# PRBonn/OverlapNet

Measured on NVIDIA H100. Metric: scan-pairs/sec (overlap+yaw) at 64x900, higher is better.
Workload: dtype f16

## Files before the change

overlapnet_b200/csrc/api.cu:

```cuda
#include "common.cuh"
#include <math.h>
#include <string.h>

using namespace ovn;

static const char* kLegNames[] = {"s_conv1", "s_conv2", "s_conv3", "s_conv3a", "s_conv4", "s_conv5",
                                  "s_conv6", "s_conv7", "s_conv8", "s_conv9", "s_conv10"};

static void set_spec(ConvSpec& L, const char* name, int kh, int kw, int sh, int sw, int cin, int cout, int relu,
                     int h_in, int w_in) {
  memset(&L, 0, sizeof(L));
  snprintf(L.name, sizeof(L.name), "%s", name);
  L.kh = kh; L.kw = kw; L.sh = sh; L.sw = sw; L.cin = cin; L.cout = cout; L.relu = relu;
  L.h_in = h_in; L.w_in = w_in;
  L.h_out = (h_in - kh) / sh + 1;
  L.w_out = (w_in - kw) / sw + 1;
}

static void slot_sizes(const ovn_handle* h, int slot, int64_t* n_kernel, int64_t* n_bias) {
  if (slot == kMaxLegLayers + 3) {
    *n_kernel = h->dense_in; *n_bias = 1;
    return;
  }
  const ConvSpec& L = slot < kMaxLegLayers ? h->leg[slot] : h->head[slot - kMaxLegLayers];
  *n_kernel = (int64_t)L.kh * L.kw * L.cin * L.cout;
  *n_bias = L.cout;
}

static __global__ void k_iota(int32_t* p, int n, int start) {
  const int i = blockIdx.x * blockDim.x + threadIdx.x;
  if (i < n) p[i] = start + i;
}

static __global__ void k_sanitize_idx(const int32_t* __restrict__ in, int32_t* __restrict__ out, int n, int64_t limit,
                                      int code, const int32_t* __restrict__ row_bad, int* __restrict__ err) {
  const int i = blockIdx.x * blockDim.x + threadIdx.x;
  if (i >= n) return;
  int64_t v = in[i];
  if (v < 0 || v >= limit) {
    atomicCAS(err, 0, code);
    v = v < 0 ? 0 : limit - 1;
  }
  if (row_bad && row_bad[v]) atomicCAS(err, 0, kErrNonFiniteOperand);
  out[i] = (int32_t)v;
}

struct PeerPtrs { int32_t* p[16]; };

static __global__ void k_peer_signal(PeerPtrs dst, int n, int value) {
  const int i = threadIdx.x;
  if (i >= n || dst.p[i] == nullptr) return;
  __threadfence_system();
  asm volatile("st.release.sys.global.s32 [%0], %1;" :: "l"(dst.p[i]), "r"(value) : "memory");
}

static __global__ void k_peer_wait(const int32_t* __restrict__ flags, int n, int skip, int value, int* __restrict__ err) {
  const int i = threadIdx.x;
  if (i >= n || i == skip) return;
  const long long t0 = clock64();
  for (;;) {
    int v;
    asm volatile("ld.acquire.sys.global.s32 %0, [%1];" : "=r"(v) : "l"(flags + i) : "memory");
    if (v >= value) break;
    if (clock64() - t0 > (1ll << 32)) { atomicCAS(err, 0, kErrPeerWait); break; }
    __nanosleep(32);
  }
}

namespace ovn {

int sanitize_indices(ovn_handle* h, const int32_t* d_in, int n, int64_t limit, int code, int32_t* d_out, cudaStream_t s,
                     const int32_t* row_bad) {
  if (n <= 0) return OVN_OK;
  k_sanitize_idx<<<(n + 255) / 256, 256, 0, s>>>(d_in, d_out, n, limit < 1 ? 1 : limit, code, row_bad, h->d_err);
  OVN_LAUNCH_CHECK(h);
  return OVN_OK;
}

int check_device_error(ovn_handle* h, cudaStream_t s) {
  if (!h->h_pinned || !h->d_err) return OVN_OK;
  int32_t* hp = &h->stage()->err;
  OVN_CUDA(h, cudaMemcpyAsync(hp, h->d_err, sizeof(int), cudaMemcpyDeviceToHost, s));
  OVN_CUDA(h, cudaStreamSynchronize(s));
  const int e = *hp;
  if (e == 0) return OVN_OK;
  OVN_CUDA(h, cudaMemsetAsync(h->d_err, 0, sizeof(int), s));
  const char* ring = nullptr;
  switch (e) {
    case kErrBadIndex: OVN_SET_ERR(h, OVN_ERR_INVALID_ARG, "a pair / candidate index is outside [0, bank_size)");
    case kErrRowNotPrepared:
      OVN_SET_ERR(h, OVN_ERR_INVALID_ARG, "resident bank: an indexed row was never passed to ovn_bank_prepare");
    case kErrNonFiniteOperand:
      OVN_SET_ERR(h, OVN_ERR_INVALID_ARG, "a feature volume value is not finite in the fp16 operands of the tensor-core "
                  "heads (NaN, inf, or |x - centre| > 65504); outputs of the call are poisoned (NaN / INT32_MIN)");
    case kErrPeerWait: OVN_SET_ERR(h, OVN_ERR_CUDA, "ovn_peer_wait timed out: a peer rank never signalled");
    case kErrInjectedFault: OVN_SET_ERR(h, OVN_ERR_CUDA, "tensor-core pipeline failed: k_conv2_wgmma: fault injected by "
                                        "OVN_DEBUG_FAULT (code %d); outputs of the call are poisoned (NaN / INT32_MIN)", e);
    case kErrDeltaLeftProducer: case kErrDeltaLeftConsumer: ring = "k_delta_conv1_wgmma: LEFT volume ring"; break;
    case kErrDeltaRightProducer: case kErrDeltaRightConsumer: ring = "k_delta_conv1_wgmma: RIGHT window ring"; break;
    case kErrDeltaW1Producer: case kErrDeltaW1Consumer: ring = "k_delta_conv1_wgmma: W1 ring"; break;
    case kErrConv2Producer: case kErrConv2Consumer: ring = "k_conv2_wgmma: o1 + W2 ring"; break;
    case kErrConv3X3Producer: case kErrConv3X3Consumer: ring = "k_conv3_wgmma: x3 ring"; break;
    case kErrConv3W3Producer: case kErrConv3W3Consumer: ring = "k_conv3_wgmma: W3 ring"; break;
    case kErrCorrRightProducer: case kErrCorrRightConsumer: ring = "k_corr_wgmma: RIGHT third ring"; break;
    case kErrCorrLeftProducer: case kErrCorrLeftConsumer: ring = "k_corr_wgmma: LEFT tile ring"; break;
  }
  if (!ring) OVN_SET_ERR(h, OVN_ERR_CUDA, "unknown device error code %d", e);
  OVN_SET_ERR(h, OVN_ERR_CUDA, "tensor-core pipeline failed: %s, %s wait timed out (code %d); outputs of the call are "
              "poisoned (NaN / INT32_MIN)", ring, e < 200 ? "producer" : "consumer", e);
}

}

extern "C" {

int ovn_abi_version(void) { return OVN_ABI_VERSION; }

const char* ovn_status_string(int status) {
  switch (status) {
    case OVN_OK: return "OVN_OK";
    case OVN_ERR_INVALID_ARG: return "OVN_ERR_INVALID_ARG";
    case OVN_ERR_BAD_CONFIG: return "OVN_ERR_BAD_CONFIG";
    case OVN_ERR_WEIGHTS: return "OVN_ERR_WEIGHTS";
    case OVN_ERR_CUDA: return "OVN_ERR_CUDA";
    case OVN_ERR_NO_DEVICE: return "OVN_ERR_NO_DEVICE";
    case OVN_ERR_CAPACITY: return "OVN_ERR_CAPACITY";
    default: return "OVN_ERR_UNKNOWN";
  }
}

void ovn_default_config(ovn_config* c) {
  if (!c) return;
  memset(c, 0, sizeof(*c));
  c->abi_version = OVN_ABI_VERSION;
  c->proj_H = 64; c->proj_W = 900;
  c->fov_up_deg = 3.0f; c->fov_down_deg = -25.0f;
  c->max_range = 50.0f;
  c->use_depth = 1; c->use_normals = 1;
  c->n_prob_channels = 0; c->use_intensity = 0;
  c->strides_layer1[0] = 2; c->strides_layer1[1] = 2;
  c->additional_unsymmetric_layer3a = 1;
  c->leg_output_width = 360;
  c->conv1size = 15;
  c->precision = OVN_PREC_F16_TC;
  c->max_batch_scans = 16;
  c->max_batch_pairs = 1101;
}

static thread_local std::string g_create_error;

const char* ovn_last_error(const ovn_handle* h) { return h ? h->last_error.c_str() : g_create_error.c_str(); }
int64_t ovn_launch_count(const ovn_handle* h) { return h ? h->launches : 0; }
int ovn_input_channels(const ovn_handle* h) { return h ? h->C : 0; }
int ovn_feature_width(const ovn_handle* h) { return h ? h->cfg.leg_output_width : 0; }
int ovn_feature_channels(const ovn_handle* h) { return h ? kFeatC : 0; }

#define CREATE_FAIL(code, ...)                              \
  do {                                                      \
    char _b[512];                                           \
    snprintf(_b, sizeof(_b), __VA_ARGS__);                  \
    g_create_error = _b;                                    \
    return (code);                                          \
  } while (0)

#define CREATE_CUDA(call)                                                              \
  do {                                                                                 \
    cudaError_t _e = (call);                                                           \
    if (_e != cudaSuccess) {                                                           \
      cudaGetLastError();                                                              \
      CREATE_FAIL(OVN_ERR_CUDA, "%s: %s", #call, cudaGetErrorString(_e));              \
    }                                                                                  \
  } while (0)

#define CREATE_ALLOC(buf, bytes)                                                       \
  do {                                                                                 \
    if ((buf).ensure(h.get(), (bytes)) != OVN_OK) CREATE_FAIL(OVN_ERR_CUDA, "ovn_create: %s", h->last_error.c_str()); \
  } while (0)

ovn_handle::~ovn_handle() {
  if (ev_bank) cudaEventDestroy(ev_bank);
  if (own_stream) cudaStreamDestroy(own_stream);
  for (auto& v : prof_ev) for (cudaEvent_t e : v) cudaEventDestroy(e);
}

int ovn_create(const ovn_config* cfg, ovn_handle** out) {
  if (!cfg || !out) CREATE_FAIL(OVN_ERR_INVALID_ARG, "ovn_create: NULL argument");
  *out = nullptr;
  if (cfg->abi_version != OVN_ABI_VERSION)
    CREATE_FAIL(OVN_ERR_INVALID_ARG, "ovn_create: abi_version %d != %d", cfg->abi_version, OVN_ABI_VERSION);
  int ndev = 0;
  if (cudaGetDeviceCount(&ndev) != cudaSuccess || ndev == 0) {
    cudaGetLastError();
    CREATE_FAIL(OVN_ERR_NO_DEVICE, "ovn_create: no CUDA device visible (this library has no CPU fallback)");
  }
  int dev = 0;
  CREATE_CUDA(cudaGetDevice(&dev));
  cudaDeviceProp prop;
  CREATE_CUDA(cudaGetDeviceProperties(&prop, dev));
  if (prop.major != 9 || prop.minor != 0)
    CREATE_FAIL(OVN_ERR_NO_DEVICE, "ovn_create: device %d is sm_%d%d; this build targets sm_90a only", dev,
                prop.major, prop.minor);
  std::unique_ptr<ovn_handle> h(new ovn_handle());
  h->cfg = *cfg;
  h->device = dev;
  h->sm_count = prop.multiProcessorCount;
  const ovn_config& c = h->cfg;
  if (c.proj_H <= 0 || c.proj_W <= 0 || c.max_batch_scans <= 0 || c.max_batch_pairs <= 0)
    CREATE_FAIL(OVN_ERR_BAD_CONFIG, "ovn_create: non-positive size in config");
  if (c.n_prob_channels != 0 && c.n_prob_channels != 3 && c.n_prob_channels != 20)
    CREATE_FAIL(OVN_ERR_BAD_CONFIG, "ovn_create: n_prob_channels must be 0, 3 or 20 (infer.py:68-73)");
  h->C = (c.use_depth ? 1 : 0) + (c.use_normals ? 3 : 0) + c.n_prob_channels + (c.use_intensity ? 1 : 0);
  if (h->C <= 0) CREATE_FAIL(OVN_ERR_BAD_CONFIG, "ovn_create: no input channel enabled");

  struct { int kh, kw, sh, sw, cout; bool opt; } T[] = {
      {5, 15, c.strides_layer1[0], c.strides_layer1[1], 16, false}, {3, 15, 2, 1, 32, false},
      {3, 15, 2, 1, 64, false},  {3, 12, 2, 1, 64, true},           {2, 9, 2, 1, 128, false},
      {1, 9, 1, 1, 128, false},  {1, 9, 1, 1, 128, false},          {1, 9, 1, 1, 128, false},
      {1, 7, 1, 1, 128, false},  {1, 5, 1, 1, 128, false},          {1, 3, 1, 1, 128, false}};
  int hh = c.proj_H, ww = c.proj_W, cc = h->C;
  h->n_leg = 0;
  h->net_ok = true;
  char nb[256];
  for (int i = 0; i < 11 && h->net_ok; ++i) {
    if (T[i].opt && !c.additional_unsymmetric_layer3a) continue;
    if (T[i].sh <= 0 || T[i].sw <= 0 || hh < T[i].kh || ww < T[i].kw) {
      snprintf(nb, sizeof(nb), "layer %s does not fit its input %dx%d", kLegNames[i], hh, ww);
      h->net_ok = false; h->net_error = nb;
      break;
    }
    set_spec(h->leg[h->n_leg], kLegNames[i], T[i].kh, T[i].kw, T[i].sh, T[i].sw, cc, T[i].cout, 1, hh, ww);
    hh = h->leg[h->n_leg].h_out; ww = h->leg[h->n_leg].w_out; cc = T[i].cout;
    h->n_leg++;
  }
  const int Wf = c.leg_output_width, s = c.conv1size;
  if (h->net_ok && (hh != 1 || ww != c.leg_output_width || cc != kFeatC)) {
    snprintf(nb, sizeof(nb), "leg output is %dx%dx%d, expected 1x%dx%d (network.yml:77)", hh, ww, cc,
             c.leg_output_width, kFeatC);
    h->net_ok = false; h->net_error = nb;
  }
  if (h->net_ok && (s <= 0 || Wf % s != 0 || Wf / s < 3)) {
    snprintf(nb, sizeof(nb), "conv1size %d must divide leg_output_width %d", s, Wf);
    h->net_ok = false; h->net_error = nb;
  }
  if (!h->net_ok) { h->n_leg = 0; *out = nullptr; }
  if (h->net_ok) {
    set_spec(h->head[0], "c_conv1", 1, s, 1, s, kFeatC, 64, 0, Wf, Wf);
    set_spec(h->head[1], "c_conv2", s, 1, s, 1, 64, 128, 1, h->head[0].h_out, h->head[0].w_out);
    set_spec(h->head[2], "c_conv3", 3, 3, 1, 1, 128, 256, 1, h->head[1].h_out, h->head[1].w_out);
    h->o1_h = h->head[0].h_out; h->o1_w = h->head[0].w_out;
    h->o2_h = h->head[1].h_out; h->o2_w = h->head[1].w_out;
    h->o3_h = h->head[2].h_out; h->o3_w = h->head[2].w_out;
    h->dense_in = h->o3_h * h->o3_w * h->head[2].cout;
    ParamLayout& P = h->params;
// ... 932 lines not shown
```

overlapnet_b200/csrc/common.cuh:

```cuda
#pragma once
#include <cuda_runtime.h>
#include <cuda_fp16.h>
#include <stddef.h>
#include <stdint.h>
#include <stdio.h>
#include <memory>
#include <string>
#include <vector>
#include <map>

#include "../../include/ovn_b200.h"

struct ovn_handle;

namespace ovn {

template <class T, bool Pinned = false>
class Buffer {
 public:
  Buffer() = default;
  Buffer(Buffer&& o) noexcept { swap(o); }
  Buffer& operator=(Buffer&& o) noexcept {
    Buffer old(std::move(o));
    swap(old);
// ... 60 lines not shown
  int64_t n_kernel[kMaxLegLayers + 4] = {};
  int64_t n_head = 0;
  int64_t n_total = 0;
};
inline int flat_slot(int i) { return i < 4 ? kMaxLegLayers + i : i - 4; }

enum GradCover { kNoGrads = 0, kHeadGrads, kNetGrads };

struct TrainState {
  Buffer<float> x4;
  Buffer<float> dx3;
  Buffer<float> corr;
  Buffer<float> overlap;
  Buffer<float> dz;
  Buffer<int32_t> yaw;
  Buffer<float> w3t;
  Buffer<float> part;
  Buffer<float> grad;
  Buffer<float> accum;
  Buffer<float> loss;
  Buffer<float> chunk_loss;
  PinnedBuffer<float> chunk_loss_host;
  GradCover grads = kNoGrads;
  Buffer<float> images;
  Buffer<float> acts;
  Buffer<float> dact[2];
  Buffer<float> dfv_part;
  Buffer<float> dcorr;
  Buffer<int32_t> pair_rows;
  Buffer<float> wt;
  int64_t net_fv_off = 0;
  int net_np = 0;
};
}

struct ovn_handle {
  ovn_config cfg;
  int device = 0;
  int sm_count = 0;
  std::string last_error;
  int64_t launches = 0;

  int C = 0;
  int n_leg = 0;
  ovn::ConvSpec leg[ovn::kMaxLegLayers];
  ovn::ConvSpec head[3];
  int o1_h = 0, o1_w = 0;
  int o2_h = 0, o2_w = 0;
  int o3_h = 0, o3_w = 0;
  int dense_in = 0;
  ovn::ParamLayout params;

  std::map<std::string, ovn::LayerWeights> host_w;
  bool weights_ready = false;
  bool net_ok = false;
  std::string net_error;

  ovn::Buffer<float> d_w[ovn::kMaxLegLayers + 4];
  ovn::Buffer<float> d_b[ovn::kMaxLegLayers + 4];

  ovn::Buffer<unsigned long long> d_keys;
  ovn::Buffer<unsigned long long> d_pair_keys;
  ovn::Buffer<uint8_t> d_pair_prune;
  ovn::Buffer<uint32_t> d_valid_words;
  ovn::Buffer<uint32_t> d_word_prefix;
  ovn::Buffer<uint32_t> d_scan_tmp;
  ovn::Buffer<float> d_act[2];
  ovn::Buffer<float> d_input;
  ovn::Buffer<float> d_o1;
  ovn::Buffer<float> d_o2;
  ovn::Buffer<float> d_G;
  ovn::Buffer<int32_t> d_cand_idx;
  ovn::Buffer<int32_t> d_idx_san;
  ovn::Buffer<int> d_err;
  cudaEvent_t ev_bank = nullptr;
  ovn::Buffer<float> d_query_fv;
  ovn::Buffer<float> d_query_overlap;
  ovn::Buffer<int32_t> d_query_yaw;
  ovn::Buffer<float> d_stage_points;
  ovn::Buffer<int64_t> d_stage_offsets;
  ovn::PinnedBuffer<uint8_t> h_pinned;
  cudaStream_t own_stream = nullptr;
  bool profiling = false;
  std::vector<cudaEvent_t> prof_ev[ovn::kProfKinds];
  std::unique_ptr<ovn::TcState, ovn::TcStateDelete> tc;
  std::unique_ptr<ovn::TrainState> train;
  int32_t train_precision = OVN_TRAIN_FP32;
  bool train_tc = false;
  bool dgrad_tc_smem = false;

  ~ovn_handle();
  ovn::StageHeader* stage() const { return reinterpret_cast<ovn::StageHeader*>(h_pinned.get()); }
  int32_t* stage_cand_idx() const { return reinterpret_cast<int32_t*>(h_pinned + sizeof(ovn::StageHeader)); }
  float* stage_overlap() const { return reinterpret_cast<float*>(stage_cand_idx() + cfg.max_batch_pairs); }
  int32_t* stage_yaw() const { return reinterpret_cast<int32_t*>(stage_overlap() + cfg.max_batch_pairs); }
};

#define OVN_SET_ERR(h, code, ...)                                 \
  do {                                                            \
    char _buf[512];                                               \
    snprintf(_buf, sizeof(_buf), __VA_ARGS__);                    \
    (h)->last_error = _buf;                                       \
    return (code);                                                \
  } while (0)

#define OVN_CUDA(h, call)                                                                   \
  do {                                                                                      \
    cudaError_t _e = (call);                                                                \
    if (_e != cudaSuccess) {                                                                \
      cudaGetLastError();                                                                   \
      OVN_SET_ERR(h, OVN_ERR_CUDA, "%s failed at %s:%d: %s", #call, __FILE__, __LINE__,     \
                  cudaGetErrorString(_e));                                                  \
    }                                                                                       \
  } while (0)

#define OVN_LAUNCH_CHECK(h)                                                                 \
  do {                                                                                      \
    (h)->launches++;                                                                        \
    cudaError_t _e = cudaGetLastError();                                                    \
    if (_e != cudaSuccess) {                                                                \
      OVN_SET_ERR(h, OVN_ERR_CUDA, "kernel launch failed at %s:%d: %s", __FILE__, __LINE__, \
                  cudaGetErrorString(_e));                                                  \
    }                                                                                       \
  } while (0)

namespace ovn {

template <class T, bool Pinned>
int Buffer<T, Pinned>::ensure(ovn_handle* h, size_t bytes, size_t reserve) {
  if (bytes <= cap_) return OVN_OK;
  *this = {};
  if (reserve < bytes) reserve = bytes;
  void* p = nullptr;
  if (Pinned) OVN_CUDA(h, cudaHostAlloc(&p, reserve, cudaHostAllocDefault));
  else OVN_CUDA(h, cudaMalloc(&p, reserve));
  p_ = static_cast<T*>(p);
  cap_ = reserve;
  return OVN_OK;
}

struct DeviceGuard {
  int prev = -1;
  bool switched = false;
  explicit DeviceGuard(const ovn_handle* h) {
    if (h && cudaGetDevice(&prev) == cudaSuccess && prev != h->device) switched = cudaSetDevice(h->device) == cudaSuccess;
  }
  ~DeviceGuard() { if (switched) cudaSetDevice(prev); }
};

enum DeviceError : int {
  kErrDeltaLeftProducer = 101, kErrDeltaLeftConsumer = 402,
  kErrDeltaRightProducer = 103, kErrDeltaRightConsumer = 404,
  kErrDeltaW1Producer = 102, kErrDeltaW1Consumer = 202,
  kErrConv2Producer = 111, kErrConv2Consumer = 211,
  kErrConv3X3Producer = 121, kErrConv3X3Consumer = 221,
  kErrConv3W3Producer = 122, kErrConv3W3Consumer = 222,
  kErrCorrRightProducer = 131, kErrCorrRightConsumer = 231,
  kErrCorrLeftProducer = 132, kErrCorrLeftConsumer = 232,
  kErrInjectedFault = 501,
  kErrBadIndex = 900,
  kErrRowNotPrepared = 901,
  kErrNonFiniteOperand = 910,
  kErrPeerWait = 950,
};

inline void prof_mark(ovn_handle* h, int kind, cudaStream_t s) {
  if (!h->profiling) return;
  cudaEvent_t e;
  if (cudaEventCreate(&e) != cudaSuccess) return;
  cudaEventRecord(e, s);
  h->prof_ev[kind].push_back(e);
}

template <class T>
int upload_vec(ovn_handle* h, Buffer<T>& dst, const std::vector<T>& v) {
  dst = {};
  const int rc = dst.ensure(h, v.size() * sizeof(T));
  if (rc != OVN_OK) return rc;
  OVN_CUDA(h, cudaMemcpy(dst, v.data(), v.size() * sizeof(T), cudaMemcpyHostToDevice));
  return OVN_OK;
}

int project_batch(ovn_handle* h, const float* d_points, const int64_t* d_offsets, int n_scans,
                  int64_t n_total, float max_range, float* d_range, float* d_vertex,
                  float* d_intensity, int32_t* d_idx, cudaStream_t s);
int normals_batch(ovn_handle* h, const float* d_range, const float* d_vertex, int n_scans,
                  float* d_normal, cudaStream_t s);
int semantic_batch(ovn_handle* h, const int32_t* d_idx, const float* d_probs,
                   const int64_t* d_offsets, int n_scans, int n_classes, float* d_out,
                   cudaStream_t s);
int preprocess_batch(ovn_handle* h, const float* d_points, const int64_t* d_offsets, int n_scans,
                     int64_t n_total, const float* d_probs, float* d_input, cudaStream_t s);
int gt_range_batch(ovn_handle* h, const float* d_points, const int64_t* d_offsets, int n_scans, int64_t n_total,
                   const double* d_pose_ref, const double* d_pose_cur_inv, float max_range, float* d_range,
                   cudaStream_t s);
int gt_overlap_count(ovn_handle* h, const float* d_ref, const float* d_cur, int n_scans, int32_t* d_counts, cudaStream_t s);
int gt_scan_radius(ovn_handle* h, const float* d_points, const int64_t* d_offsets, int n_scans, double* d_radius,
                   cudaStream_t s);
int gt_pairs_count(ovn_handle* h, const float* d_points, const int64_t* h_offsets, int n_ref, const double* d_pose_ref,
                   const double* d_radius, const float* d_cur_range, const double* d_pose_cur_inv, int n_cur,
                   float max_range, int tile_cur, int tile_ref, int32_t* d_counts, int64_t ld_counts,
                   int64_t* d_n_pruned, cudaStream_t s);
int pack_input(ovn_handle* h, const float* d_depth, const float* d_normal, const float* d_prob,
               const float* d_intensity, int n_scans, float* d_input, cudaStream_t s);

int leg_forward_fp32(ovn_handle* h, const float* d_input, int n, float* d_fv, cudaStream_t s);
int heads_forward_fp32(ovn_handle* h, const float* d_bank, const float* d_query,
                       const int32_t* d_left, const int32_t* d_right, int n, float* d_overlap,
                       int32_t* d_yaw, float* d_corr, cudaStream_t s);

constexpr int kMaxSumParts = 64;

struct GradChunks {
  int n = 1;
  int off[kMaxSumParts + 1] = {};
  float* grad = nullptr;
  int64_t stride = 0;
  float* loss = nullptr;
  __host__ __device__ int size(int c) const { return off[c + 1] - off[c]; }
};

int train_alloc(ovn_handle* h);
int head_gradients_fp32(ovn_handle* h, const float* d_bank, const int32_t* left, const int32_t* right, int np,
                        const float* d_gt_overlap, const int32_t* d_gt_orientation, float min_overlap,
                        const GradChunks& ch, cudaStream_t s);
int net_gradients_fp32(ovn_handle* h, const float* d_images, const int32_t* left, const int32_t* right, int np,
                       const float* d_gt_overlap, const int32_t* d_gt_orientation, float min_overlap,
                       float* d_fv_grad, const GradChunks& ch, cudaStream_t s);
int net_max_pairs(const ovn_handle* h);
int64_t train_workspace_bytes(const ovn_handle* h, bool whole_network, int np);
int copy_net_volumes_fp32(ovn_handle* h, float* d_out, cudaStream_t s);
int adagrad_sum_fp32(ovn_handle* h, bool whole_network, const float* d_parts, int n_parts, const float* h_weights,
                     float lr, cudaStream_t s);
int gather_images(ovn_handle* h, const float* d_images, int64_t n_images, const int32_t* d_rows,
                  const int32_t* d_shift, const float* d_rot, int n, float* d_out, cudaStream_t s);

int corr_forward_fp32(ovn_handle* h, const float* d_bank, const float* d_query, const int32_t* left,
                      const int32_t* right, int np, int32_t* d_yaw, float* d_corr, cudaStream_t s);

int leg_forward_tc(ovn_handle* h, const float* d_input, int n, float* d_fv, cudaStream_t s);
int heads_forward_tc(ovn_handle* h, const float* d_bank, const float* d_query,
                     const int32_t* d_left, const int32_t* d_right, int n, float* d_overlap,
                     int32_t* d_yaw, float* d_corr, cudaStream_t s);
int tc_pack_weights(ovn_handle* h);
int tc_bank_prepare(ovn_handle* h, const float* d_bank, int64_t capacity, int64_t first, int64_t count, cudaStream_t s);
int tc_bank_release(ovn_handle* h, const float* d_bank);
int tc_set_center(ovn_handle* h, const float* h_mu);
int tc_get_center(ovn_handle* h, float* h_mu, int32_t* is_set);
int tc_calibrate(ovn_handle* h, const float* d_volume, cudaStream_t s);
int tc_copy_heads_stage(ovn_handle* h, int stage, int64_t first, int64_t count, float* d_out, cudaStream_t s);
int64_t tc_heads_stage_pairs(const ovn_handle* h);
int sanitize_indices(ovn_handle* h, const int32_t* d_in, int n, int64_t limit, int code, int32_t* d_out, cudaStream_t s,
                     const int32_t* row_bad = nullptr);
int check_device_error(ovn_handle* h, cudaStream_t s);

}
```

overlapnet_b200/csrc/hopper.cuh:

```cuda
#pragma once
#include <cuda_runtime.h>
#include <stdint.h>

namespace hopper {

__device__ __forceinline__ uint32_t smem_u32(const void* p) { return (uint32_t)__cvta_generic_to_shared(p); }

__device__ __forceinline__ void mbar_init(uint64_t* bar, uint32_t count) {
  asm volatile("mbarrier.init.shared::cta.b64 [%0], %1;" :: "r"(smem_u32(bar)), "r"(count) : "memory");
}
__device__ __forceinline__ void mbar_fence_init() { asm volatile("fence.mbarrier_init.release.cluster;" ::: "memory"); }
__device__ __forceinline__ void mbar_arrive(uint64_t* bar) {
  asm volatile("{\n\t.reg .b64 st;\n\tmbarrier.arrive.shared::cta.b64 st, [%0];\n\t}\n" :: "r"(smem_u32(bar)) : "memory");
}
__device__ __forceinline__ void mbar_arrive_expect_tx(uint64_t* bar, uint32_t bytes) {
  asm volatile("{\n\t.reg .b64 st;\n\tmbarrier.arrive.expect_tx.shared::cta.b64 st, [%0], %1;\n\t}\n"
               :: "r"(smem_u32(bar)), "r"(bytes) : "memory");
}
__device__ __forceinline__ bool mbar_try_wait(uint64_t* bar, uint32_t parity) {
  uint32_t ok;
  asm volatile("{\n\t.reg .pred p;\n\tmbarrier.try_wait.parity.shared::cta.b64 p, [%1], %2;\n\tselp.u32 %0, 1, 0, p;\n\t}\n"
               : "=r"(ok) : "r"(smem_u32(bar)), "r"(parity) : "memory");
  return ok != 0;
}
__device__ __forceinline__ bool mbar_wait(uint64_t* bar, uint32_t parity, long long max_cycles) {
  if (mbar_try_wait(bar, parity)) return true;
  const long long t0 = clock64();
  while (!mbar_try_wait(bar, parity))
    if (clock64() - t0 > max_cycles) return false;
  return true;
}
constexpr long long kMbarWaitCycles = 1ll << 28;

template <int D>
struct MbarRing {
  uint64_t full[D], empty[D];
  __device__ __forceinline__ void init(uint32_t consumer_arrivals) {
    for (int s = 0; s < D; ++s) { mbar_init(&full[s], 1); mbar_init(&empty[s], consumer_arrivals); }
  }
  static __device__ __forceinline__ uint32_t slot(uint32_t i) { return i % D; }
  static __device__ __forceinline__ uint32_t parity(uint32_t i) { return (i / D) & 1; }
  __device__ __forceinline__ bool acquire(uint32_t i, uint32_t bytes) {
    if (!mbar_wait(&empty[slot(i)], parity(i) ^ 1, kMbarWaitCycles)) return false;
    mbar_arrive_expect_tx(&full[slot(i)], bytes);
    return true;
  }
  __device__ __forceinline__ bool try_acquire(uint32_t i, uint32_t bytes) {
    if (!mbar_try_wait(&empty[slot(i)], parity(i) ^ 1)) return false;
    mbar_arrive_expect_tx(&full[slot(i)], bytes);
    return true;
  }
  __device__ __forceinline__ uint64_t* bar(uint32_t i) { return &full[slot(i)]; }
  __device__ __forceinline__ bool wait(uint32_t i) { return mbar_wait(&full[slot(i)], parity(i), kMbarWaitCycles); }
  __device__ __forceinline__ void release(uint32_t i) {
    __syncwarp();
    if ((threadIdx.x & 31) == 0) mbar_arrive(&empty[slot(i)]);
  }
};

#define PIPE_WAIT(ok, code) \
  if (!(ok)) { atomicExch(err, (code)); goto done; }
#define INFLIGHT_WAIT(ok, code) \
  if (!failed && !(ok)) { atomicExch(err, (code)); failed = true; }

__device__ __forceinline__ void named_bar_sync(int id, int count) {
  asm volatile("bar.sync %0, %1;" :: "r"(id), "r"(count) : "memory");
}

template <uint32_t N>
__device__ __forceinline__ void setmaxnreg_dec() { asm volatile("setmaxnreg.dec.sync.aligned.u32 %0;" :: "n"(N)); }
template <uint32_t N>
__device__ __forceinline__ void setmaxnreg_inc() { asm volatile("setmaxnreg.inc.sync.aligned.u32 %0;" :: "n"(N)); }

__device__ __forceinline__ void bulk_g2s(void* smem_dst, const void* gmem_src, uint32_t bytes, uint64_t* bar) {
  asm volatile("cp.async.bulk.shared::cluster.global.mbarrier::complete_tx::bytes [%0], [%1], %2, [%3];"
               :: "r"(smem_u32(smem_dst)), "l"(gmem_src), "r"(bytes), "r"(smem_u32(bar)) : "memory");
}

constexpr uint32_t kNoSwizzle = 0, kSwizzle128B = 1;
__device__ __forceinline__ uint64_t desc_kmajor(uint32_t smem_addr, uint32_t lbo, uint32_t sbo, uint32_t layout) {
  return (uint64_t)((smem_addr >> 4) & 0x3FFF) | ((uint64_t)((lbo >> 4) & 0x3FFF) << 16) |
         ((uint64_t)((sbo >> 4) & 0x3FFF) << 32) | ((uint64_t)layout << 62);
}
__device__ __forceinline__ void wgmma_fence() { asm volatile("wgmma.fence.sync.aligned;" ::: "memory"); }
__device__ __forceinline__ void wgmma_commit() { asm volatile("wgmma.commit_group.sync.aligned;" ::: "memory"); }
template <int N>
__device__ __forceinline__ void wgmma_wait() { asm volatile("wgmma.wait_group.sync.aligned %0;" :: "n"(N) : "memory"); }

__device__ __forceinline__ void wgmma_m64n64k16_rs(float (&d)[32], const uint32_t (&a)[4], uint64_t b_desc) {
  asm volatile(
      "{\n\t.reg .pred p;\n\tsetp.ne.b32 p, %37, 0;\n\t"
      "wgmma.mma_async.sync.aligned.m64n64k16.f32.f16.f16 {%0, %1, %2, %3, %4, %5, %6, %7, %8, %9, %10, %11, %12, %13, %14, %15, %16, %17, %18, %19, %20, %21, %22, %23, %24, %25, %26, %27, %28, %29, %30, %31}, {%32, %33, %34, %35}, %36, p, 1, 1, 0;\n\t}\n"
      : "+f"(d[0]), "+f"(d[1]), "+f"(d[2]), "+f"(d[3]), "+f"(d[4]), "+f"(d[5]), "+f"(d[6]), "+f"(d[7]), "+f"(d[8]), "+f"(d[9]), "+f"(d[10]), "+f"(d[11]), "+f"(d[12]), "+f"(d[13]), "+f"(d[14]), "+f"(d[15]), "+f"(d[16]), "+f"(d[17]), "+f"(d[18]), "+f"(d[19]), "+f"(d[20]), "+f"(d[21]), "+f"(d[22]), "+f"(d[23]), "+f"(d[24]), "+f"(d[25]), "+f"(d[26]), "+f"(d[27]), "+f"(d[28]), "+f"(d[29]), "+f"(d[30]), "+f"(d[31])
      : "r"(a[0]), "r"(a[1]), "r"(a[2]), "r"(a[3]), "l"(b_desc), "r"(1)
      : "memory");
}

__device__ __forceinline__ void wgmma_m64n128k16_ss(float (&d)[64], uint64_t a_desc, uint64_t b_desc) {
  asm volatile(
      "{\n\t.reg .pred p;\n\tsetp.ne.b32 p, %66, 0;\n\t"
      "wgmma.mma_async.sync.aligned.m64n128k16.f32.f16.f16 {%0, %1, %2, %3, %4, %5, %6, %7, %8, %9, %10, %11, %12, %13, %14, %15, %16, %17, %18, %19, %20, %21, %22, %23, %24, %25, %26, %27, %28, %29, %30, %31, %32, %33, %34, %35, %36, %37, %38, %39, %40, %41, %42, %43, %44, %45, %46, %47, %48, %49, %50, %51, %52, %53, %54, %55, %56, %57, %58, %59, %60, %61, %62, %63}, %64, %65, p, 1, 1, 0, 0;\n\t}\n"
      : "+f"(d[0]), "+f"(d[1]), "+f"(d[2]), "+f"(d[3]), "+f"(d[4]), "+f"(d[5]), "+f"(d[6]), "+f"(d[7]), "+f"(d[8]), "+f"(d[9]), "+f"(d[10]), "+f"(d[11]), "+f"(d[12]), "+f"(d[13]), "+f"(d[14]), "+f"(d[15]), "+f"(d[16]), "+f"(d[17]), "+f"(d[18]), "+f"(d[19]), "+f"(d[20]), "+f"(d[21]), "+f"(d[22]), "+f"(d[23]), "+f"(d[24]), "+f"(d[25]), "+f"(d[26]), "+f"(d[27]), "+f"(d[28]), "+f"(d[29]), "+f"(d[30]), "+f"(d[31]), "+f"(d[32]), "+f"(d[33]), "+f"(d[34]), "+f"(d[35]), "+f"(d[36]), "+f"(d[37]), "+f"(d[38]), "+f"(d[39]), "+f"(d[40]), "+f"(d[41]), "+f"(d[42]), "+f"(d[43]), "+f"(d[44]), "+f"(d[45]), "+f"(d[46]), "+f"(d[47]), "+f"(d[48]), "+f"(d[49]), "+f"(d[50]), "+f"(d[51]), "+f"(d[52]), "+f"(d[53]), "+f"(d[54]), "+f"(d[55]), "+f"(d[56]), "+f"(d[57]), "+f"(d[58]), "+f"(d[59]), "+f"(d[60]), "+f"(d[61]), "+f"(d[62]), "+f"(d[63])
      : "l"(a_desc), "l"(b_desc), "r"(1)
      : "memory");
}

}
```

overlapnet_b200/csrc/network_tc.cu:

```cuda
#include "common.cuh"
#include "hopper.cuh"

#include <cuda_fp16.h>
#include <stddef.h>
#include <stdlib.h>

namespace ovn {

using namespace hopper;

constexpr int WF = 360;
constexpr int CF = 128;
constexpr int S15 = 15;
constexpr int NB = 24;
constexpr int PAIR_ROWS = NB * NB;
constexpr int K4_PITCH = CF;

struct TcState {
  Buffer<__half> w1p;
  Buffer<__half> w2p;
  Buffer<__half> w3p;
  Buffer<float> b2eff;
  Buffer<__half> wres[kMaxLegLayers];
  Buffer<__half> actp[2];
  Buffer<float> leg_part;
  Buffer<__half> l16;
  Buffer<__half> r16;
  Buffer<__half> o1;
  Buffer<__half> x3;
  Buffer<float> partial;
  Buffer<__half> lc;
  Buffer<__half> rc;
  Buffer<float> corr_part;
  const float* pb_key = nullptr;
  int64_t pb_rows = 0;
  Buffer<__half> pb_l16;
  Buffer<__half> pb_lc;
  Buffer<int32_t> pb_bad;
  Buffer<float> mu;
  bool mu_set = false;
  Buffer<float> mu_o1;
  Buffer<float> mu_x3;
  Buffer<float> b2base;
  Buffer<float> b3eff;
  bool act_set = false;
  int64_t rows_pad = 0;
  int64_t last_n = 0;
};

void TcStateDelete::operator()(TcState* t) const { delete t; }

__host__ __device__ __forceinline__ int k4_pos(int r, int c) {
  const int k = c & 31;
  return (((c >> 5) ^ (r & 1)) << 5) + ((k & 7) >> 1) * 8 + (k >> 3) * 2 + (k & 1);
}

__device__ __forceinline__ bool h2_nonfinite(__half2 v) {
  const uint32_t b = *reinterpret_cast<const uint32_t*>(&v);
  return (b & 0x7c00u) == 0x7c00u || (b & 0x7c000000u) == 0x7c000000u;
}

__global__ void __launch_bounds__(256)
k_gather_rows_f16(const float* __restrict__ bank, const int32_t* __restrict__ idx, int n, const float* __restrict__ mu,
                  int row_shift, __half* __restrict__ out, int* __restrict__ err, int32_t* __restrict__ row_bad) {
  const int64_t per = (int64_t)WF * CF / 4;
  const int64_t i = (int64_t)blockIdx.x * blockDim.x + threadIdx.x;
  if (i >= (int64_t)n * per) return;
  const int p = (int)(i / per);
  const int64_t e = i % per;
  const int64_t row = idx ? idx[p] : p;
  const int r = (int)(e / (CF / 4)), c4 = (int)(e % (CF / 4));
  int64_t rs = r + row_shift;
  if (rs >= WF) rs -= WF;
  const float4 v = __ldg(reinterpret_cast<const float4*>(bank + (row * WF + rs) * CF) + c4);
  const float4 m = __ldg(reinterpret_cast<const float4*>(mu) + c4);
  __half2 a = __floats2half2_rn(v.x - m.x, v.y - m.y), b = __floats2half2_rn(v.z - m.z, v.w - m.w);
  if (h2_nonfinite(a) || h2_nonfinite(b)) {
    if (row_bad) row_bad[p] = 1;
    else atomicCAS(err, 0, kErrNonFiniteOperand);
  }
  __half* o = out + ((int64_t)p * WF + r) * K4_PITCH;
  *reinterpret_cast<uint32_t*>(o + k4_pos(r, 4 * c4)) = *reinterpret_cast<uint32_t*>(&a);
  *reinterpret_cast<uint32_t*>(o + k4_pos(r, 4 * c4 + 2)) = *reinterpret_cast<uint32_t*>(&b);
}

__global__ void __launch_bounds__(1024)
k_channel_mean(const float* __restrict__ bank, const int32_t* __restrict__ idx, int n, float* __restrict__ mu) {
  __shared__ float part[8][CF];
  const int c = threadIdx.x & (CF - 1), g = threadIdx.x >> 7;
  float acc = 0.f;
  for (int v = 0; v < n; ++v) {
    const float* vol = bank + (int64_t)(idx ? idx[v] : v) * WF * CF;
    for (int r = g; r < WF; r += 8) acc += __ldg(vol + (int64_t)r * CF + c);
  }
  part[g][c] = acc;
  __syncthreads();
  if (g == 0) {
    float t = 0.f;
    for (int k = 0; k < 8; ++k) t += part[k][c];
    mu[c] = __half2float(__float2half_rn(t / (float)((int64_t)n * WF)));
  }
}

constexpr int K4_STEPS = 60;

__host__ __device__ __forceinline__ size_t o1_chunk_offset(int64_t m, int di, int c8) {
  const int r = (int)(m & 127);
  return ((size_t)((m >> 7) * S15 + di) * 128 + r) * 64 + (size_t)((c8 ^ (r & 7)) * 8);
}

struct LegArgs {
  const __half* A; int64_t a_pitch;
  int runs_per_img, in_img_planes, in_run_planes;
  int kh, kw, c8in;
  const __half* Bp;
  const float* bias; int n_valid;
  int64_t M;
  __half* out_planes; int64_t out_pitch; int out_run_planes;
  float* out_f32;
  int n_split; float* part;
};

constexpr int C6_LROWS = 64, C6_RROWS = 128;
constexpr int C6_LT = 6, C6_RT = 3;
constexpr int C6_L_BYTES = 2 * 16 * C6_LROWS * 16;
constexpr int C6_R_BYTES = 2 * 16 * C6_RROWS * 16;
constexpr int C6_VOL_L_BYTES = C6_LT * C6_L_BYTES;
constexpr int C6_VOL_R_BYTES = C6_RT * C6_R_BYTES;

template <int TR, int NT>
__global__ void __launch_bounds__(256)
k_pack_corr(const float* __restrict__ bank, const int32_t* __restrict__ idx, int n, __half* __restrict__ out,
            int* __restrict__ err, int32_t* __restrict__ row_bad) {
  const int64_t i = (int64_t)blockIdx.x * blockDim.x + threadIdx.x;
  const int64_t per = 16 * NT * TR;
  if (i >= (int64_t)n * per) return;
  const int p = (int)(i / per);
  int r = (int)(i % per);
  const int vrow = r % (NT * TR); r /= NT * TR;
  const int pl = r;
  const int tile = vrow / TR, row = vrow % TR;
  float v[8];
  if (vrow < WF) {
    const int64_t src = (idx ? idx[p] : p);
    const float4 a = __ldg(reinterpret_cast<const float4*>(bank + (src * WF + vrow) * CF + pl * 8));
    const float4 b = __ldg(reinterpret_cast<const float4*>(bank + (src * WF + vrow) * CF + pl * 8 + 4));
    v[0] = a.x; v[1] = a.y; v[2] = a.z; v[3] = a.w; v[4] = b.x; v[5] = b.y; v[6] = b.z; v[7] = b.w;
  } else {
#pragma unroll
    for (int e = 0; e < 8; ++e) v[e] = 0.f;
  }
  __half hi[8], lo[8];
#pragma unroll
  for (int e = 0; e < 8; ++e) {
    hi[e] = __float2half_rn(v[e]);
    lo[e] = __float2half_rn(v[e] - __half2float(hi[e]));
  }
  bool bad = false;
#pragma unroll
  for (int e = 0; e < 8; e += 2) bad |= h2_nonfinite(__halves2half2(hi[e], hi[e + 1]));
  if (bad) {
    if (row_bad) row_bad[p] = 1;
    else atomicCAS(err, 0, kErrNonFiniteOperand);
  }
  __half* base = out + ((size_t)p * NT + tile) * (2 * 16 * TR * 8);
  *reinterpret_cast<uint4*>(base + ((size_t)pl * TR + row) * 8) = *reinterpret_cast<const uint4*>(hi);
  *reinterpret_cast<uint4*>(base + ((size_t)(16 + pl) * TR + row) * 8) = *reinterpret_cast<const uint4*>(lo);
}

constexpr int MMA_THREADS = 128;
constexpr int MMA_ROWS = 64;

__device__ __forceinline__ void mma16816(float (&d)[4], uint32_t a0, uint32_t a1, uint32_t a2, uint32_t a3,
                                         uint32_t b0, uint32_t b1) {
  asm volatile("mma.sync.aligned.m16n8k16.row.col.f32.f16.f16.f32 {%0,%1,%2,%3}, {%4,%5,%6,%7}, {%8,%9}, {%0,%1,%2,%3};"
               : "+f"(d[0]), "+f"(d[1]), "+f"(d[2]), "+f"(d[3])
               : "r"(a0), "r"(a1), "r"(a2), "r"(a3), "r"(b0), "r"(b1));
}

__device__ __forceinline__ uint32_t ld_h2(const __half* p) { return __ldg(reinterpret_cast<const unsigned int*>(p)); }

__device__ __forceinline__ uint32_t absdiff_h2(uint32_t a, uint32_t b) {
  const __half2 d = __hsub2(*reinterpret_cast<const __half2*>(&a), *reinterpret_cast<const __half2*>(&b));
  return *reinterpret_cast<const uint32_t*>(&d) & 0x7fff7fffu;
}

__device__ __forceinline__ uint32_t pack_h2(float a, float b) {
  const __half2 h = __floats2half2_rn(a, b);
  return *reinterpret_cast<const uint32_t*>(&h);
}

constexpr int K4_WG = 3;
constexpr int K4_THREADS = (K4_WG + 1) * 128;
constexpr uint32_t K4_REG_PRODUCER = 32, K4_REG_CONSUMER = 160;
constexpr int K4_GROUP = 5;
constexpr int K4_NGROUPS = K4_STEPS / K4_GROUP;
static_assert(S15 % K4_GROUP == 0, "a W1 group within one 32-channel chunk");
constexpr int K4_RING = 4;
constexpr int K4_BSLICE = 4096;
constexpr uint32_t K4_VOL_BYTES = WF * K4_PITCH * 2;
constexpr uint32_t K4_RWIN_BYTES = S15 * K4_PITCH * 2;

struct K4Smem {
  __half L[WF * K4_PITCH];
  __half Rw[2][S15 * K4_PITCH];
  __half B[K4_RING][K4_GROUP * K4_BSLICE / 2];
  MbarRing<K4_RING> w1;
  MbarRing<1> left;
  MbarRing<2> right;
};
static_assert(sizeof(K4Smem) <= 232448, "k_delta_conv1_wgmma shared memory");
static_assert(offsetof(K4Smem, B) % 16 == 0 && offsetof(K4Smem, Rw) % 16 == 0, "bulk-copy alignment");

struct Share { int64_t begin, end; };
__device__ __forceinline__ Share work_share(int64_t n, uint32_t part, uint32_t parts) {
  return {n * part / parts, n * (part + 1) / parts};
}

__global__ void __launch_bounds__(K4_THREADS, 1)
k_delta_conv1_wgmma(const __half* __restrict__ L16, const int32_t* __restrict__ l_idx, const __half* __restrict__ R16,
                    int r_per_pair, const __half* __restrict__ W1p, const float* __restrict__ mu_o1,
                    __half* __restrict__ o1, int n_pairs, int* __restrict__ err) {
  extern __shared__ __align__(128) uint8_t smem_raw[];
  K4Smem& S = *reinterpret_cast<K4Smem*>(smem_raw);
  const int tid = threadIdx.x, warp = tid >> 5, lane = tid & 31;
  const Share share = work_share((int64_t)n_pairs * NB, blockIdx.x, gridDim.x);
  const int u_begin = (int)share.begin, u_end = (int)share.end;
  if (tid == 0) {
    S.w1.init(K4_WG * 4);
    S.left.init(K4_WG * 4);
    S.right.init(K4_WG * 4);
    mbar_fence_init();
  }
  __syncthreads();

  if (warp >= K4_WG * 4) {
    setmaxnreg_dec<K4_REG_PRODUCER>();
    if (warp == K4_WG * 4 && lane == 0) {
      uint32_t pi = 0, gi = 0, ui = 0;
      for (int u = u_begin; u < u_end; ++u, ++ui) {
        const int p = u / NB, jb = u - p * NB;
        if (u == u_begin || jb == 0) {
          PIPE_WAIT(S.left.acquire(pi, K4_VOL_BYTES), kErrDeltaLeftProducer);
          bulk_g2s(S.L, L16 + (size_t)(l_idx ? l_idx[p] : p) * WF * K4_PITCH, K4_VOL_BYTES, S.left.bar(pi));
          ++pi;
        }
        PIPE_WAIT(S.right.acquire(ui, K4_RWIN_BYTES), kErrDeltaRightProducer);
        bulk_g2s(S.Rw[S.right.slot(ui)], R16 + (r_per_pair ? (size_t)p * WF * K4_PITCH : 0) + (size_t)jb * S15 * K4_PITCH,
                 K4_RWIN_BYTES, S.right.bar(ui));
        for (int grp = 0; grp < K4_NGROUPS; ++grp, ++gi) {
          PIPE_WAIT(S.w1.acquire(gi, K4_GROUP * K4_BSLICE), kErrDeltaW1Producer);
          bulk_g2s(S.B[S.w1.slot(gi)], W1p + (size_t)grp * K4_GROUP * (K4_BSLICE / 2), K4_GROUP * K4_BSLICE, S.w1.bar(gi));
        }
      }
    }
  } else {
    setmaxnreg_inc<K4_REG_CONSUMER>();
    const int wg = warp >> 2, wi = warp & 3, g = lane >> 2, t = lane & 3;
    int rows[2][2];
#pragma unroll
    for (int tt = 0; tt < 2; ++tt) {
      const int r = (wg + 3 * tt) * 64 + wi * 16 + g;
      rows[tt][0] = r;
      rows[tt][1] = r + 8;
    }
    const uint32_t b_base = smem_u32(S.B[0]);
    uint32_t pi = 0, gi = 0, ui = 0;
    for (int u = u_begin; u < u_end; ++u, ++ui) {
      const int p = u / NB, jb = u - p * NB;
      if (u == u_begin || jb == 0) { PIPE_WAIT(S.left.wait(pi), kErrDeltaLeftConsumer); ++pi; }
      const uint32_t wb = S.right.slot(ui);
      PIPE_WAIT(S.right.wait(ui), kErrDeltaRightConsumer);
      float acc[2][32];
#pragma unroll
      for (int j = 0; j < 8; ++j) {
        const float m0 = __half2float(__float2half_rn(-__ldg(mu_o1 + j * 8 + 2 * t)));
        const float m1 = __half2float(__float2half_rn(-__ldg(mu_o1 + j * 8 + 2 * t + 1)));
#pragma unroll
        for (int tt = 0; tt < 2; ++tt) {
          acc[tt][4 * j + 0] = m0; acc[tt][4 * j + 1] = m1;
          acc[tt][4 * j + 2] = m0; acc[tt][4 * j + 3] = m1;
        }
      }
      uint32_t Lr[2][2][4];
#pragma unroll 1
      for (int grp = 0; grp < K4_NGROUPS; ++grp, ++gi) {
        const int cc = grp / 3, dj0 = (grp - 3 * cc) * K4_GROUP;
        if (dj0 == 0) {
#pragma unroll
          for (int tt = 0; tt < 2; ++tt)
#pragma unroll
            for (int h = 0; h < 2; ++h) {
              const int r = rows[tt][h] < WF ? rows[tt][h] : WF - 1;
              const uint4 v = *reinterpret_cast<const uint4*>(S.L + r * K4_PITCH + ((cc ^ (r & 1)) << 5) + 8 * t);
              Lr[tt][h][0] = v.x; Lr[tt][h][1] = v.y; Lr[tt][h][2] = v.z; Lr[tt][h][3] = v.w;
            }
        }
        const uint32_t s = S.w1.slot(gi);
        const uint64_t bdesc = desc_kmajor(b_base + s * (K4_GROUP * K4_BSLICE), 1024, 128, kNoSwizzle);
        const int par = (jb + dj0) & 1;
        const __half* rw = S.Rw[wb] + dj0 * K4_PITCH + 8 * t;
        const __half* rp[2] = {rw + ((cc ^ par) << 5), rw + ((cc ^ par ^ 1) << 5)};
        uint4 rv = *reinterpret_cast<const uint4*>(rp[0]);
        PIPE_WAIT(S.w1.wait(gi), kErrDeltaW1Consumer);
        uint32_t A[2][2][4];
#pragma unroll
        for (int sl = 0; sl < K4_GROUP; ++sl)
#pragma unroll
          for (int kk = 0; kk < 2; ++kk) {
            const uint32_t r0 = kk ? rv.z : rv.x, r1 = kk ? rv.w : rv.y;
#pragma unroll
            for (int tt = 0; tt < 2; ++tt) {
              A[tt][kk][0] = absdiff_h2(Lr[tt][0][2 * kk], r0);
              A[tt][kk][1] = absdiff_h2(Lr[tt][1][2 * kk], r0);
              A[tt][kk][2] = absdiff_h2(Lr[tt][0][2 * kk + 1], r1);
              A[tt][kk][3] = absdiff_h2(Lr[tt][1][2 * kk + 1], r1);
            }
            wgmma_fence();
#pragma unroll
            for (int tt = 0; tt < 2; ++tt)
              wgmma_m64n64k16_rs(acc[tt], A[tt][kk], bdesc + ((sl * K4_BSLICE + kk * 2048) >> 4));
            wgmma_commit();
            if (kk == 1 && sl + 1 < K4_GROUP) rv = *reinterpret_cast<const uint4*>(rp[(sl + 1) & 1] + (sl + 1) * K4_PITCH);
            wgmma_wait<1>();
          }
        wgmma_wait<0>();
        S.w1.release(gi);
      }
      S.right.release(ui);
      if (jb == NB - 1 || u == u_end - 1) S.left.release(pi - 1);
      const int64_t mrow = (int64_t)p * PAIR_ROWS + jb * NB;
#pragma unroll
      for (int tt = 0; tt < 2; ++tt)
#pragma unroll
        for (int h = 0; h < 2; ++h) {
          const int i = rows[tt][h];
          if (i >= WF) continue;
          const int ibk = i / S15, di = i - ibk * S15;
#pragma unroll
          for (int j = 0; j < 8; ++j)
            *reinterpret_cast<uint32_t*>(o1 + o1_chunk_offset(mrow + ibk, di, j) + 2 * t) =
                pack_h2(acc[tt][4 * j + 2 * h], acc[tt][4 * j + 2 * h + 1]);
        }
    }
  }
done:
  return;
}

constexpr int TC_WG = 2;
constexpr int TC_THREADS = TC_WG * 128 + 32;
constexpr int TC_ROWS = TC_WG * 128;
constexpr uint32_t C2_TILE = 128 * 64 * 2;
constexpr int C2_RING = 3;

struct C2Smem {
  __half A[C2_RING][TC_WG][C2_TILE / 2];
  __half B[C2_RING][2][C2_TILE / 2];
  MbarRing<C2_RING> ring;
};
constexpr size_t C2_SMEM = sizeof(C2Smem) + 1024;
static_assert(C2_SMEM <= 232448, "k_conv2_wgmma shared memory");
static_assert(offsetof(C2Smem, B) % 1024 == 0 && C2_TILE % 1024 == 0, "SWIZZLE_128B tiles on 1024-byte boundaries");

__global__ void __launch_bounds__(TC_THREADS, 1)
k_conv2_wgmma(const __half* __restrict__ o1, const __half* __restrict__ W2s, const float* __restrict__ bias2,
              const float* __restrict__ mu_x3, __half* __restrict__ x3, int64_t out_pitch, int64_t M, int fault,
              int* __restrict__ err) {
  if (fault) {
    if (threadIdx.x == 0 && blockIdx.x == 0) atomicExch(err, kErrInjectedFault);
    return;
  }
  extern __shared__ __align__(128) uint8_t smem_raw[];
  C2Smem& S = *reinterpret_cast<C2Smem*>(smem_raw + ((1024 - (smem_u32(smem_raw) & 1023)) & 1023));
  const int tid = threadIdx.x, warp = tid >> 5, lane = tid & 31;
  const Share tiles = work_share((M + TC_ROWS - 1) / TC_ROWS, blockIdx.x, gridDim.x);
  if (tid == 0) {
    S.ring.init(TC_WG * 4);
    mbar_fence_init();
  }
  __syncthreads();

  if (warp == TC_WG * 4) {
    if (lane == 0) {
      uint32_t gi = 0;
      for (int64_t tile = tiles.begin; tile < tiles.end; ++tile)
        for (int di = 0; di < S15; ++di, ++gi) {
          const uint32_t s = S.ring.slot(gi);
          PIPE_WAIT(S.ring.acquire(gi, 4 * C2_TILE), kErrConv2Producer);
          for (int h = 0; h < TC_WG; ++h)
            bulk_g2s(S.A[s][h], o1 + ((size_t)(tile * TC_WG + h) * S15 + di) * (C2_TILE / 2), C2_TILE, S.ring.bar(gi));
          bulk_g2s(S.B[s], W2s + (size_t)di * C2_TILE, 2 * C2_TILE, S.ring.bar(gi));
        }
    }
  } else {
    const int wg = warp >> 2, wi = warp & 3, g = lane >> 2, t = lane & 3;
    uint32_t gi = 0;
    bool failed = false;
    for (int64_t tile = tiles.begin; tile < tiles.end; ++tile) {
      float acc[2][64];
#pragma unroll
      for (int sub = 0; sub < 2; ++sub)
#pragma unroll
        for (int e = 0; e < 64; ++e) acc[sub][e] = 0.f;
#pragma unroll 1
      for (int di = 0; di < S15; ++di, ++gi) {
        const uint32_t s = S.ring.slot(gi);
        INFLIGHT_WAIT(S.ring.wait(gi), kErrConv2Consumer);
        const uint32_t a_base = smem_u32(S.A[s][wg]), b_base = smem_u32(S.B[s][0]);
        wgmma_fence();
#pragma unroll
        for (int kk = 0; kk < 4; ++kk)
#pragma unroll
          for (int part = 0; part < 2; ++part) {
            const uint64_t bd = desc_kmajor(b_base + part * C2_TILE + kk * 32, 16, 1024, kSwizzle128B);
#pragma unroll
            for (int sub = 0; sub < 2; ++sub)
              wgmma_m64n128k16_ss(acc[sub], desc_kmajor(a_base + sub * (C2_TILE / 2) + kk * 32, 16, 1024, kSwizzle128B), bd);
          }
        wgmma_commit();
        wgmma_wait<1>();
        if (di > 0) S.ring.release(gi - 1);
      }
      wgmma_wait<0>();
      if (failed) goto done;
      S.ring.release(gi - 1);
#pragma unroll
      for (int sub = 0; sub < 2; ++sub)
#pragma unroll
        for (int h = 0; h < 2; ++h) {
          const int64_t m = tile * TC_ROWS + wg * 128 + sub * 64 + wi * 16 + g + 8 * h;
          if (m >= M) continue;
#pragma unroll
          for (int j = 0; j < 16; ++j) {
            const int n = j * 8 + 2 * t;
            const float a = fmaxf(acc[sub][4 * j + 2 * h] + __ldg(bias2 + n), 0.f) - __ldg(mu_x3 + n);
            const float b = fmaxf(acc[sub][4 * j + 2 * h + 1] + __ldg(bias2 + n + 1), 0.f) - __ldg(mu_x3 + n + 1);
            *reinterpret_cast<uint32_t*>(x3 + ((size_t)j * out_pitch + m) * 8 + 2 * t) = pack_h2(a, b);
          }
        }
    }
  }
done:
  return;
}

constexpr int C3_AROWS = TC_ROWS + 2 * NB + 2;
constexpr uint32_t C3_PLANE = C3_AROWS * 16;
constexpr uint32_t C3_SLAB = 4 * 128 * 16;
constexpr int C3_GROUP = 2;
constexpr int C3_NSTAGES = 36 / C3_GROUP;
constexpr int C3_RING = 4;

struct C3Smem {
  __half A[2][16 * C3_PLANE / 2];
  __half B[C3_RING][C3_GROUP * C3_SLAB / 2];
  MbarRing<C3_RING> w3;
  MbarRing<2> x3;
};
static_assert(sizeof(C3Smem) <= 232448, "k_conv3_wgmma shared memory");
static_assert(offsetof(C3Smem, B) % 16 == 0 && C3_PLANE % 16 == 0, "bulk-copy alignment");

__global__ void __launch_bounds__(TC_THREADS, 1)
k_conv3_wgmma(const __half* __restrict__ X3, int64_t a_pitch, const __half* __restrict__ W3p, const float* __restrict__ bias,
              int64_t M, const float* __restrict__ wd, float* __restrict__ partial, int* __restrict__ err) {
  extern __shared__ __align__(128) uint8_t smem_raw[];
  C3Smem& S = *reinterpret_cast<C3Smem*>(smem_raw);
  const int tid = threadIdx.x, warp = tid >> 5, lane = tid & 31;
  const Share tiles = work_share(2 * ((M + TC_ROWS - 1) / TC_ROWS), blockIdx.x, gridDim.x);
  if (tid == 0) {
    S.w3.init(TC_WG * 4);
    S.x3.init(TC_WG * 4);
    mbar_fence_init();
  }
  __syncthreads();

  if (warp == TC_WG * 4) {
    if (lane == 0) {
      const uint32_t nt = (uint32_t)(tiles.end - tiles.begin);
      uint32_t ai = 0, gi = 0;
      for (uint32_t ti = 0; ti < nt; ++ti) {
        const int nh = (int)((tiles.begin + ti) & 1);
        for (int st = 0; st < C3_NSTAGES; ++st, ++gi) {
          while (ai < nt && ai <= ti + 1) {
            if (ai > ti) {
              if (!S.x3.try_acquire(ai, 16 * C3_PLANE)) break;
            } else {
              PIPE_WAIT(S.x3.acquire(ai, 16 * C3_PLANE), kErrConv3X3Producer);
            }
            const int64_t r0 = ((tiles.begin + ai) >> 1) * TC_ROWS;
            for (int pl = 0; pl < 16; ++pl)
              bulk_g2s(S.A[S.x3.slot(ai)] + pl * (C3_PLANE / 2), X3 + ((size_t)pl * a_pitch + r0) * 8, C3_PLANE, S.x3.bar(ai));
            ++ai;
          }
          PIPE_WAIT(S.w3.acquire(gi, C3_GROUP * C3_SLAB), kErrConv3W3Producer);
          bulk_g2s(S.B[S.w3.slot(gi)], W3p + ((size_t)nh * 36 + st * C3_GROUP) * (C3_SLAB / 2), C3_GROUP * C3_SLAB,
// ... 1001 lines not shown
```

Before: 199,600.

## Stage conv1 outputs in shared memory and store via bulk async copies

The delta-conv1 consumers now write their fp16 accumulator tiles into a swizzled shared-memory staging buffer instead of scattering 4-byte stores directly to global memory. A second producer warp then issues cp.async.bulk shared-to-global copies per row block, and an mbarrier handshake guards the single staging slot. The aim is to replace many uncoalesced global stores with bulk TMA stores and to overlap output writeback with the next unit's compute. In exchange there is extra shared memory, a proxy fence, and a single-buffer wait that can stall consumers until the previous copy has been read out.

```diff
diff --git a/overlapnet_b200/csrc/api.cu b/overlapnet_b200/csrc/api.cu
--- a/overlapnet_b200/csrc/api.cu
+++ b/overlapnet_b200/csrc/api.cu
@@ -99,6 +99,7 @@
     case kErrDeltaLeftProducer: case kErrDeltaLeftConsumer: ring = "k_delta_conv1_wgmma: LEFT volume ring"; break;
     case kErrDeltaRightProducer: case kErrDeltaRightConsumer: ring = "k_delta_conv1_wgmma: RIGHT window ring"; break;
     case kErrDeltaW1Producer: case kErrDeltaW1Consumer: ring = "k_delta_conv1_wgmma: W1 ring"; break;
+    case kErrDeltaO1Producer: case kErrDeltaO1Consumer: ring = "k_delta_conv1_wgmma: o1 staging"; break;
     case kErrConv2Producer: case kErrConv2Consumer: ring = "k_conv2_wgmma: o1 + W2 ring"; break;
     case kErrConv3X3Producer: case kErrConv3X3Consumer: ring = "k_conv3_wgmma: x3 ring"; break;
     case kErrConv3W3Producer: case kErrConv3W3Consumer: ring = "k_conv3_wgmma: W3 ring"; break;
diff --git a/overlapnet_b200/csrc/common.cuh b/overlapnet_b200/csrc/common.cuh
--- a/overlapnet_b200/csrc/common.cuh
+++ b/overlapnet_b200/csrc/common.cuh
@@ -236,6 +236,7 @@
   kErrDeltaLeftProducer = 101, kErrDeltaLeftConsumer = 402,
   kErrDeltaRightProducer = 103, kErrDeltaRightConsumer = 404,
   kErrDeltaW1Producer = 102, kErrDeltaW1Consumer = 202,
+  kErrDeltaO1Producer = 104, kErrDeltaO1Consumer = 405,
   kErrConv2Producer = 111, kErrConv2Consumer = 211,
   kErrConv3X3Producer = 121, kErrConv3X3Consumer = 221,
   kErrConv3W3Producer = 122, kErrConv3W3Consumer = 222,
diff --git a/overlapnet_b200/csrc/hopper.cuh b/overlapnet_b200/csrc/hopper.cuh
--- a/overlapnet_b200/csrc/hopper.cuh
+++ b/overlapnet_b200/csrc/hopper.cuh
@@ -35,8 +35,8 @@
 template <int D>
 struct MbarRing {
   uint64_t full[D], empty[D];
-  __device__ __forceinline__ void init(uint32_t consumer_arrivals) {
-    for (int s = 0; s < D; ++s) { mbar_init(&full[s], 1); mbar_init(&empty[s], consumer_arrivals); }
+  __device__ __forceinline__ void init(uint32_t consumer_arrivals, uint32_t producer_arrivals = 1) {
+    for (int s = 0; s < D; ++s) { mbar_init(&full[s], producer_arrivals); mbar_init(&empty[s], consumer_arrivals); }
   }
   static __device__ __forceinline__ uint32_t slot(uint32_t i) { return i % D; }
   static __device__ __forceinline__ uint32_t parity(uint32_t i) { return (i / D) & 1; }
@@ -55,6 +55,14 @@
   __device__ __forceinline__ void release(uint32_t i) {
     __syncwarp();
     if ((threadIdx.x & 31) == 0) mbar_arrive(&empty[slot(i)]);
+  }
+  __device__ __forceinline__ void release_thread(uint32_t i) { mbar_arrive(&empty[slot(i)]); }
+  __device__ __forceinline__ bool wait_free(uint32_t i) {
+    return mbar_wait(&empty[slot(i)], parity(i) ^ 1, kMbarWaitCycles);
+  }
+  __device__ __forceinline__ void publish(uint32_t i) {
+    __syncwarp();
+    if ((threadIdx.x & 31) == 0) mbar_arrive(&full[slot(i)]);
   }
 };
 
@@ -76,6 +84,17 @@
   asm volatile("cp.async.bulk.shared::cluster.global.mbarrier::complete_tx::bytes [%0], [%1], %2, [%3];"
                :: "r"(smem_u32(smem_dst)), "l"(gmem_src), "r"(bytes), "r"(smem_u32(bar)) : "memory");
 }
+
+__device__ __forceinline__ void bulk_s2g(void* gmem_dst, const void* smem_src, uint32_t bytes) {
+  asm volatile("cp.async.bulk.global.shared::cta.bulk_group [%0], [%1], %2;"
+               :: "l"(gmem_dst), "r"(smem_u32(smem_src)), "r"(bytes) : "memory");
+}
+__device__ __forceinline__ void bulk_commit() { asm volatile("cp.async.bulk.commit_group;" ::: "memory"); }
+template <int N>
+__device__ __forceinline__ void bulk_wait_read() { asm volatile("cp.async.bulk.wait_group.read %0;" :: "n"(N) : "memory"); }
+template <int N>
+__device__ __forceinline__ void bulk_wait() { asm volatile("cp.async.bulk.wait_group %0;" :: "n"(N) : "memory"); }
+__device__ __forceinline__ void fence_proxy_async_smem() { asm volatile("fence.proxy.async.shared::cta;" ::: "memory"); }
 
 constexpr uint32_t kNoSwizzle = 0, kSwizzle128B = 1;
 __device__ __forceinline__ uint64_t desc_kmajor(uint32_t smem_addr, uint32_t lbo, uint32_t sbo, uint32_t layout) {
diff --git a/overlapnet_b200/csrc/network_tc.cu b/overlapnet_b200/csrc/network_tc.cu
--- a/overlapnet_b200/csrc/network_tc.cu
+++ b/overlapnet_b200/csrc/network_tc.cu
@@ -104,9 +104,11 @@
 
 constexpr int K4_STEPS = 60;
 
+__host__ __device__ __forceinline__ size_t o1_row_offset(int64_t m, int di) {
+  return ((size_t)((m >> 7) * S15 + di) * 128 + (size_t)(m & 127)) * 64;
+}
 __host__ __device__ __forceinline__ size_t o1_chunk_offset(int64_t m, int di, int c8) {
-  const int r = (int)(m & 127);
-  return ((size_t)((m >> 7) * S15 + di) * 128 + r) * 64 + (size_t)((c8 ^ (r & 7)) * 8);
+  return o1_row_offset(m, di) + (size_t)((c8 ^ (int)(m & 7)) * 8);
 }
 
 struct LegArgs {
@@ -200,17 +202,21 @@
 constexpr int K4_BSLICE = 4096;
 constexpr uint32_t K4_VOL_BYTES = WF * K4_PITCH * 2;
 constexpr uint32_t K4_RWIN_BYTES = S15 * K4_PITCH * 2;
+constexpr int K4_O1S_PITCH = NB * 64 + 8;
 
 struct K4Smem {
   __half L[WF * K4_PITCH];
   __half Rw[2][S15 * K4_PITCH];
   __half B[K4_RING][K4_GROUP * K4_BSLICE / 2];
+  __half O1s[S15 * K4_O1S_PITCH];
   MbarRing<K4_RING> w1;
   MbarRing<1> left;
   MbarRing<2> right;
+  MbarRing<1> o1s;
 };
 static_assert(sizeof(K4Smem) <= 232448, "k_delta_conv1_wgmma shared memory");
-static_assert(offsetof(K4Smem, B) % 16 == 0 && offsetof(K4Smem, Rw) % 16 == 0, "bulk-copy alignment");
+static_assert(offsetof(K4Smem, B) % 16 == 0 && offsetof(K4Smem, Rw) % 16 == 0 && offsetof(K4Smem, O1s) % 16 == 0 &&
+              K4_O1S_PITCH * 2 % 16 == 0, "bulk-copy alignment");
 
 struct Share { int64_t begin, end; };
 __device__ __forceinline__ Share work_share(int64_t n, uint32_t part, uint32_t parts) {
@@ -230,6 +236,7 @@
     S.w1.init(K4_WG * 4);
     S.left.init(K4_WG * 4);
     S.right.init(K4_WG * 4);
+    S.o1s.init(1, K4_WG * 4);
     mbar_fence_init();
   }
   __syncthreads();
@@ -253,6 +260,24 @@
           bulk_g2s(S.B[S.w1.slot(gi)], W1p + (size_t)grp * K4_GROUP * (K4_BSLICE / 2), K4_GROUP * K4_BSLICE, S.w1.bar(gi));
         }
       }
+    } else if (warp == K4_WG * 4 + 1 && lane == 0) {
+      uint32_t ui = 0;
+      for (int u = u_begin; u < u_end; ++u, ++ui) {
+        const int p = u / NB, jb = u - p * NB;
+        const int64_t m0 = (int64_t)p * PAIR_ROWS + jb * NB;
+        const int n0 = min(NB, 128 - (int)(m0 & 127));
+        if (!S.o1s.wait(ui)) { atomicExch(err, kErrDeltaO1Producer); break; }
+#pragma unroll 1
+        for (int di = 0; di < S15; ++di) {
+          const __half* src = S.O1s + di * K4_O1S_PITCH;
+          bulk_s2g(o1 + o1_row_offset(m0, di), src, n0 * 128);
+          if (n0 < NB) bulk_s2g(o1 + o1_row_offset(m0 + n0, di), src + n0 * 64, (NB - n0) * 128);
+        }
+        bulk_commit();
+        bulk_wait_read<0>();
+        S.o1s.release_thread(ui);
+      }
+      bulk_wait<0>();
     }
   } else {
     setmaxnreg_inc<K4_REG_CONSUMER>();
@@ -329,7 +354,7 @@
       }
       S.right.release(ui);
       if (jb == NB - 1 || u == u_end - 1) S.left.release(pi - 1);
-      const int64_t mrow = (int64_t)p * PAIR_ROWS + jb * NB;
+      if (!S.o1s.wait_free(ui)) { atomicExch(err, kErrDeltaO1Consumer); goto done; }
 #pragma unroll
       for (int tt = 0; tt < 2; ++tt)
 #pragma unroll
@@ -337,11 +362,14 @@
           const int i = rows[tt][h];
           if (i >= WF) continue;
           const int ibk = i / S15, di = i - ibk * S15;
+          __half* st = S.O1s + di * K4_O1S_PITCH + ibk * 64 + 2 * t;
 #pragma unroll
           for (int j = 0; j < 8; ++j)
-            *reinterpret_cast<uint32_t*>(o1 + o1_chunk_offset(mrow + ibk, di, j) + 2 * t) =
+            *reinterpret_cast<uint32_t*>(st + ((j ^ (ibk & 7)) << 3)) =
                 pack_h2(acc[tt][4 * j + 2 * h], acc[tt][4 * j + 2 * h + 1]);
         }
+      fence_proxy_async_smem();
+      S.o1s.publish(ui);
     }
   }
 done:
```

New measurement: 208,600 (median of 6 runs). 1.05x the previous value.
